# SimFlowCFD/RapidCFD-dev

Hardware: AMD Instinct MI355X
Metric: PCG iterations/s + HBM GB/s on 10M-cell lduMatrix at 1/2/4/8 MI355X (higher is better)
Workload: dtype f64

## Files before the change

### rapidcfd-dev_amd/csrc/engine.hip

```cpp
#include <hip/hip_ext.h>
#include "../../include/mi_ldu.h"
#include "kernels.hip.hpp"
#include "tiling.hpp"
#include "host_parallel.hpp"

#include <algorithm>
#include <atomic>
#include <cstdio>
#include <cstdlib>
#include <cstring>
#include <condition_variable>
#include <functional>
#include <map>
#include <set>
#include <mutex>
#include <string>
#include <thread>
#include <vector>

using namespace mi;
constexpr int HALO_NV = 6;

namespace {

thread_local std::string g_err;
int fail(int code, const std::string& msg) { g_err = msg; return code; }

#define HIPCHK(expr)                                                                          \
    do {                                                                                      \
        hipError_t e__ = (expr);                                                              \
        if (e__ != hipSuccess)                                                                \
            return fail(MI_ERR_DEVICE, std::string(#expr) + ": " + hipGetErrorString(e__));   \
    } while (0)
#define MICHK(expr) do { int r__ = (expr); if (r__ != MI_OK) return r__; } while (0)

template <class T>
struct DevBuf {
    T* p = nullptr;
    size_t n = 0;
    DevBuf() = default;
    DevBuf(const DevBuf&) = delete;
    DevBuf& operator=(const DevBuf&) = delete;
    ~DevBuf() { release(); }
    void release() { if (p) { (void)hipFree(p); p = nullptr; n = 0; } }
    int alloc(size_t count)
    {
        if (count == n && p) return MI_OK;
        release();
        if (hipMalloc((void**)&p, (count ? count : 1) * sizeof(T)) != hipSuccess) { p = nullptr; return fail(MI_ERR_ALLOC, "hipMalloc failed"); }
        n = count;
        return MI_OK;
    }
    template <class A>
    int upload(const std::vector<T, A>& v, hipStream_t s)
    {
        MICHK(alloc(v.size()));
        if (!v.empty()) HIPCHK(hipMemcpyAsync(p, v.data(), v.size() * sizeof(T), hipMemcpyHostToDevice, s));
        return MI_OK;
    }
};

int env_int(const char* name, int def)
{
    const char* v = getenv(name);
    return (v && *v) ? atoi(v) : def;
}

}

struct mi_ctx_s {
    int device = 0;
    hipStream_t stream = nullptr;
    bool ownStream = false;
    DevBuf<double> partial;
    DevBuf<double> scalars;
    DevBuf<PcgState> state;
    PcgState* hostState = nullptr;
    double* hostScal = nullptr;
    hipEvent_t ev0 = nullptr, ev1 = nullptr;
    hipStream_t sideStream = nullptr;
    hipEvent_t evSideGo = nullptr, evSideDone = nullptr;
    int amulBS = 0;
    int tileFlags = 0;
    int xcdRows = 1;
    int persist = 0;
    int nCU = 0;
    bool coarseLevelBuild = false;
    bool keepSlotTables = false;
    int attachEvents = 1;
    int fusePerm = 1;
    int deferPsi = 1;
    int fuseFinal = 0;
    int pcgFuseTest = 0;
    int pcgFuseRP = -1;
    int pcgPersist = 1;
    int64_t stats[12] = {};
    int persistGrid = 0;
    int persistShared = 0;
    int persistCoop = -1;
    uint64_t faultEpoch = 0;
    int winDirect = 1;
    int gamgGraphAttached = 1;
    int multiPipe = 1;
    int fusePrologue = 1;
    int pairAT = 1;
    struct mi_matrix_s* session = nullptr;
    int pcgBatch = 16, pcgGraph = -1, pbicgHostStepped = 0, gamgDeviceInvert = -1, gamgAlwaysAgglomerate = 0, gamgGraph = 1, gamgFuse = 1;
    std::set<const void*> ldsAttrSet;
    std::map<std::pair<const void*, size_t>, int> occCache;
};

struct mi_addr_s {
    mi_ctx_s* ctx = nullptr;
    TileLayout L;
    DevBuf<int32_t> e2c, c2e, tileCellStart, tileSlotStart, tileIfaceSlot0, tileHaloStart, haloCell, tileSliceStart, sliceEntryStart;
    DevBuf<uint32_t> entries, entries16;
    DevBuf<int32_t> sliceEntryStart16, tileSbStart;
    DevBuf<uint16_t> slotBase;
    bool compact = false;
    DevBuf<int32_t> slotFace, extSlot, interiorTiles, boundaryTiles, patchFaceCellsE, faceSlot, lowerAddr, upperAddr;
    DevBuf<int32_t> ownerStartC, losortStartC, losortC;
    DevBuf<uint32_t> row16; DevBuf<uint16_t> losort16; DevBuf<int32_t> rowEsc, rowEscStart;
    struct RowPlan { bool tiles = false; int bs = 256, blocks = 0, maxFaces = 0, capForced = 0; } rowPlan[2];
    DevBuf<double> relaxD0, relaxSumOff;
    DevBuf<uint8_t> setMask; DevBuf<double> setVal;
    Table<int32_t> lowerHost, upperHost;
    int32_t nInterior = 0, nBoundary = 0, nLocalPatches = 0;
    Table<char> patchIsLocal;
    DevBuf<int32_t> ifaceNbrCaller;
    DevBuf<int32_t> haloSrc;
    Table<Table<int32_t>> patchFaceCellsHost, patchNbrCellsHost;
    int64_t nEntries = 0, nHaloTot = 0;
    struct AmiPatch {
        int32_t patch = 0, nbrPatch = 0, n = 0, extOff = 0;
        Table<int32_t> transports, partCount;
        int32_t transport = -1, nPartner = 0;
        DevBuf<int32_t> start, cellE, ownE; DevBuf<double> w; bool hasLow = false;
        Table<int32_t> hStart, hAddr; Table<double> hW, hMagSf;
    };
    Table<AmiPatch*> ami;
    bool amiRemote = false;
    ~mi_addr_s() { for (AmiPatch* q : ami) delete q; }
    bool identity = false;
    const int32_t* perm() const { return identity ? nullptr : e2c.p; }
};

struct mi_dpcg_s { double *psi = nullptr, *src = nullptr, *pA = nullptr, *wA = nullptr, *rA = nullptr, *scal = nullptr, *send = nullptr; int precond = 0; };

struct mi_matrix_s {
    mi_addr_s* addr = nullptr;
    mi_dpcg_s dp;
    DevBuf<double> diagE, upE, lowE, rD, sumAE;
    bool asym = false, bound = false, rDValid = false, sumAValid = false;
    Table<double> patchFactor;
    uint64_t epoch = 0;
    Table<DevBuf<double>*> work;
    DevBuf<double> hist, tilePartial;
    DevBuf<PcgState> mstate; DevBuf<double> mpartial, mhist, mtilePartial; PcgState* mhostState = nullptr;
    DevBuf<double> persistScratch;
    uint64_t persistFaultEpoch = 0;
    DevBuf<double> persistZ;
    int histLen = 0;
    int pcgIt = 0, pcgPrecond = MI_PRECOND_DIAGONAL;
    bool pcgActive = false;
    bool pcgPReady = false;
    DevBuf<unsigned int> fusedBar;
    unsigned int fusedGen = 0;
    Table<hipEvent_t> evPool;
    hipGraphExec_t pcgGraph = nullptr;
    struct { int precond = -1, batch = 0, histLen = 0; const void* hist = nullptr; const void* psi = nullptr; } pcgGraphKey;
    bool gateDone = false;
    double *proY2 = nullptr, *proY3 = nullptr;
    const double *callerX = nullptr, *callerB = nullptr; double* callerY = nullptr;
    hipEvent_t kevStart = nullptr, kevStop = nullptr;
    struct mi_dpcg_comm_s* dpc = nullptr;
    DevBuf<double> sendBuf, dscal;
    ~mi_matrix_s();
    int vec(size_t k, double** out)
    {
        while (work.size() <= k) work.push_back(new DevBuf<double>());
        const size_t need = (size_t)addr->L.nCells + (size_t)addr->L.nExt;
        if (work[k]->n != need) {
            MICHK(work[k]->alloc(need));
            HIPCHK(hipMemsetAsync(work[k]->p, 0, need * sizeof(double), addr->ctx->stream));
        }
        *out = work[k]->p;
        return MI_OK;
    }
};

bool comm_remote(const mi_matrix_s* m);
bool comm_attached(const mi_matrix_s* m);
bool comm_any_ami(const mi_matrix_s* m);
bool comm_any_factor(const mi_matrix_s* m);
bool comm_any_compact(const mi_matrix_s* m);
bool matrix_has_factor(const mi_matrix_s* m);
void comm_inherit_factor_flag(mi_matrix_s* level, const mi_matrix_s* fine);
int64_t comm_n_global(const mi_matrix_s* m);
int comm_exchange_start(mi_matrix_s* m, const double* send, double* vec);
int comm_exchange_wait(mi_matrix_s* m);
int comm_allreduce(mi_matrix_s* m, double* dev, size_t n);
bool peer_halo_ready(const mi_matrix_s* m);
int peer_exchange_push(mi_matrix_s* m, const double* x);
int peer_exchange_pull(mi_matrix_s* m, double* x);
int peer_exchange_push_n(mi_matrix_s* m, int nv, const double* const* xs);
int peer_exchange_pull_n(mi_matrix_s* m, int nv, double* const* xs);
bool peer_win_direct(mi_matrix_s* m);
int peer_check(mi_matrix_s* m);
int dpcg_flush_if_fused(mi_matrix_s* m);
bool peer_reduce_ready(const mi_matrix_s* m);
int peer_globalize(mi_matrix_s* m, int n, double* const* P);
int pcg_solve_attached(mi_matrix_s* m, double* psi_io, const double* source, const mi_solver_controls* ctl, int precond,
                       mi_solver_perf* perf, double* hist_host, int32_t hist_len);

extern "C" const char* mi_last_error(void) { return g_err.c_str(); }

extern "C" int mi_device_available(void)
{
    int n = 0;
    if (hipGetDeviceCount(&n) != hipSuccess || n <= 0) return 0;
    hipDeviceProp_t prop;
    if (hipGetDeviceProperties(&prop, 0) != hipSuccess) return 0;
    return strncmp(prop.gcnArchName, "gfx950", 6) == 0 ? 1 : 0;
}

extern "C" int mi_ctx_create(int device, void* hip_stream, mi_ctx_t* out)
{
    if (!out) return fail(MI_ERR_ARG, "out is NULL");
    int n = 0;
    const hipError_t e0 = hipGetDeviceCount(&n);
    if (e0 != hipSuccess || n <= 0)
        return fail(MI_ERR_DEVICE, std::string("no HIP device visible: the engine has no CPU fallback (hipGetDeviceCount: ") + hipGetErrorString(e0) + ", " + std::to_string(n) + " devices)");
    if (device < 0 || device >= n) return fail(MI_ERR_ARG, "device index out of range");
    HIPCHK(hipSetDevice(device));
    hipDeviceProp_t prop;
    HIPCHK(hipGetDeviceProperties(&prop, device));
    if (strncmp(prop.gcnArchName, "gfx950", 6) != 0)
        return fail(MI_ERR_DEVICE, std::string("engine is built for gfx950 only, found ") + prop.gcnArchName);
    mi_ctx_s* c = new mi_ctx_s();
    c->device = device;
    if (hip_stream) c->stream = (hipStream_t)hip_stream;
    else { if (hipStreamCreate(&c->stream) != hipSuccess) { delete c; return fail(MI_ERR_DEVICE, "hipStreamCreate failed"); } c->ownStream = true; }
    int r = c->partial.alloc(4 * RG);
    if (r == MI_OK) r = c->scalars.alloc(16);
    if (r == MI_OK) r = c->state.alloc(1);
    if (r != MI_OK) { delete c; return r; }
    if (hipHostMalloc((void**)&c->hostState, sizeof(PcgState)) != hipSuccess ||
        hipHostMalloc((void**)&c->hostScal, 16 * sizeof(double)) != hipSuccess ||
        hipEventCreate(&c->ev0) != hipSuccess || hipEventCreate(&c->ev1) != hipSuccess) {
        delete c; return fail(MI_ERR_DEVICE, "pinned host / event allocation failed");
    }
    c->tileFlags = env_int("MI_TILE_FLAGS", 1);
    c->attachEvents = env_int("MI_EVENT_ATTACH", 1);
    c->persist = env_int("MI_TILE_PERSIST", 0);
    c->xcdRows = env_int("MI_XCD_ROWS", 1);
    c->deferPsi = env_int("MI_PCG_DEFER_PSI", 1);
    c->fusePerm = env_int("MI_FUSE_PERM", 1);
    { hipDeviceProp_t pr; if (hipGetDeviceProperties(&pr, device) == hipSuccess) c->nCU = pr.multiProcessorCount; }
    c->pairAT = env_int("MI_PBICG_PAIR", 1);
    c->fusePrologue = env_int("MI_FUSE_PROLOGUE", 1);
    c->multiPipe = env_int("MI_MULTI_PIPE", 1);
    c->winDirect = env_int("MI_WIN_DIRECT", 1); c->gamgGraphAttached = env_int("MI_GAMG_GRAPH_ATTACHED", 1);
    c->pcgPersist = env_int("MI_PCG_PERSIST", 1);
    c->pcgFuseRP = env_int("MI_PCG_FUSE_RP", 1) != 0 ? -1 : 0;
    c->persistGrid = env_int("MI_PERSIST_GRID", 0);
    c->persistShared = env_int("MI_PERSIST_SHARED", 0);
    c->fuseFinal = env_int("MI_PCG_FUSE_FINAL", 0);
    c->amulBS = env_int("MI_AMUL_BS", 0);
    c->pcgBatch = env_int("MI_PCG_BATCH", 16);
    if (c->pcgBatch < 1) c->pcgBatch = 1;
    c->pcgGraph = env_int("MI_PCG_GRAPH", -1); c->pbicgHostStepped = env_int("MI_PBICG_HOST_STEPPED", 0);
    c->gamgDeviceInvert = env_int("MI_GAMG_DEVICE_INVERT", -1); c->gamgAlwaysAgglomerate = env_int("MI_GAMG_ALWAYS_AGGLOMERATE", 0); c->gamgGraph = env_int("MI_GAMG_GRAPH", 1); c->gamgFuse = env_int("MI_GAMG_FUSE", 1);
    if (c->amulBS != 256 && c->amulBS != 512 && c->amulBS != 1024) c->amulBS = 0;
    *out = c;
    return MI_OK;
}

extern "C" int mi_ctx_destroy(mi_ctx_t c)
{
    if (!c) return MI_OK;
    (void)hipSetDevice(c->device);
    (void)hipStreamSynchronize(c->stream);
    if (c->hostState) (void)hipHostFree(c->hostState);
    if (c->hostScal) (void)hipHostFree(c->hostScal);
    if (c->ev0) (void)hipEventDestroy(c->ev0);
    if (c->ev1) (void)hipEventDestroy(c->ev1);
    if (c->sideStream) { (void)hipStreamSynchronize(c->sideStream); (void)hipStreamDestroy(c->sideStream); }
    if (c->evSideGo) (void)hipEventDestroy(c->evSideGo);
    if (c->evSideDone) (void)hipEventDestroy(c->evSideDone);
    if (c->ownStream) (void)hipStreamDestroy(c->stream);
    delete c;
    return MI_OK;
}

extern "C" int mi_ctx_synchronize(mi_ctx_t c)
{
    if (!c) return fail(MI_ERR_ARG, "ctx is NULL");
    HIPCHK(hipStreamSynchronize(c->stream));
    return MI_OK;
}

extern "C" int mi_ctx_set_option(mi_ctx_t c, const char* name, int32_t value)
{
    if (!c || !name) return fail(MI_ERR_ARG, "mi_ctx_set_option: bad argument");
    if (std::string(name) == "pcg_persist") { c->pcgPersist = value; return MI_OK; }
    if (std::string(name) == "pcg_fuse_rp") { c->pcgFuseRP = value != 0 ? -1 : 0; return MI_OK; }
    if (std::string(name) == "pcg_fuse_test") { c->pcgFuseTest = value; return MI_OK; }
    if (std::string(name) == "fuse_prologue") { c->fusePrologue = value; return MI_OK; }
    if (std::string(name) == "win_direct") { c->winDirect = value; return MI_OK; }
    if (std::string(name) == "gamg_graph_attached") { c->gamgGraphAttached = value; return MI_OK; }
    return fail(MI_ERR_ARG, "mi_ctx_set_option: unknown option");
}

extern "C" int mi_ctx_stat(mi_ctx_t c, int32_t which, int64_t* out)
{
    if (!c || !out || which < 0 || which >= (int32_t)(sizeof(c->stats) / sizeof(c->stats[0]))) return fail(MI_ERR_ARG, "mi_ctx_stat: bad argument");
    *out = c->stats[which];
    return MI_OK;
}

extern "C" int mi_addr_create_coupled(mi_ctx_t ctx, int32_t n_cells, int32_t n_faces,
                                      const int32_t* lower, const int32_t* upper, int32_t n_patches,
                                      const int32_t* patch_sizes, const int32_t* const* patch_face_cells,
                                      const int32_t* const* patch_nbr_cells, mi_addr_t* out);

extern "C" int mi_addr_create(mi_ctx_t ctx, int32_t n_cells, int32_t n_faces,
                              const int32_t* lower, const int32_t* upper, int32_t n_patches,
                              const int32_t* patch_sizes, const int32_t* const* patch_face_cells,
                              mi_addr_t* out)
{
    return mi_addr_create_coupled(ctx, n_cells, n_faces, lower, upper, n_patches, patch_sizes, patch_face_cells, nullptr, out);
}

static int addr_create_impl(mi_ctx_t ctx, int32_t n_cells, int32_t n_faces, const int32_t* lower, const int32_t* upper, int32_t n_patches,
                            const int32_t* patch_sizes, const int32_t* const* patch_face_cells, const int32_t* const* patch_nbr_cells,
                            bool ordered, int32_t n_tiles, const int32_t* tile_cell_start, mi_addr_t* out, TileLayout* prebuilt);

extern "C" int mi_addr_create_coupled(mi_ctx_t ctx, int32_t n_cells, int32_t n_faces,
                                      const int32_t* lower, const int32_t* upper, int32_t n_patches,
                                      const int32_t* patch_sizes, const int32_t* const* patch_face_cells,
                                      const int32_t* const* patch_nbr_cells, mi_addr_t* out)
{
    return addr_create_impl(ctx, n_cells, n_faces, lower, upper, n_patches, patch_sizes, patch_face_cells, patch_nbr_cells, false, 0, nullptr, out, nullptr);
}

extern "C" int mi_addr_create_ordered(mi_ctx_t ctx, int32_t n_cells, int32_t n_faces, const int32_t* lower, const int32_t* upper,
                                      int32_t n_patches, const int32_t* patch_sizes, const int32_t* const* patch_face_cells,
                                      const int32_t* const* patch_nbr_cells, int32_t n_tiles, const int32_t* tile_cell_start, mi_addr_t* out)
{
    if (tile_cell_start && n_tiles <= 0) return fail(MI_ERR_ARG, "mi_addr_create_ordered: n_tiles must be positive when tile_cell_start is given");
    return addr_create_impl(ctx, n_cells, n_faces, lower, upper, n_patches, patch_sizes, patch_face_cells, patch_nbr_cells, true, n_tiles, tile_cell_start, out, nullptr);
}

namespace {
struct AdoptedMesh {
    Table<int32_t> cellMap, faceMap, lower, upper, tileStart;
    Table<uint8_t> flipped;
    Table<Table<int32_t>> patchFaceCells, patchNbrCells;
};
std::string adopt_engine_order(int32_t n_cells, int32_t n_faces, const int32_t* lower, const int32_t* upper, int32_t n_patches, const int32_t* patch_sizes,
                               const int32_t* const* patch_face_cells, const int32_t* const* patch_nbr_cells, AdoptedMesh& M)
{
    TileLayout L;
    TileParams prm;
    prm.tileCells = env_int("MI_TILE_CELLS", 0) > 0 ? env_int("MI_TILE_CELLS", 0) : 1024;
    prm.slotCap = env_int("MI_TILE_SLOTS", 4094);
    prm.reorder = env_int("MI_TILE_REORDER", -1);
    prm.compact = false;
    const std::string err = build_tile_layout(n_cells, n_faces, lower, upper, n_patches, patch_sizes, patch_face_cells, prm, L, patch_nbr_cells);
    if (!err.empty()) return err;
    M.cellMap = L.e2c; M.tileStart = L.tileCellStart;
    const Table<int32_t>& o2n = L.c2e;
    Table<int32_t> lo((size_t)n_faces), up((size_t)n_faces);
    Table<uint8_t> fl((size_t)n_faces);
    for (int32_t f = 0; f < n_faces; ++f) {
        const int32_t a = o2n[(size_t)lower[f]], b = o2n[(size_t)upper[f]];
        fl[(size_t)f] = a > b; lo[(size_t)f] = a < b ? a : b; up[(size_t)f] = a < b ? b : a;
    }
    Table<int32_t> byUp((size_t)n_faces), cnt((size_t)n_cells + 1, 0);
    for (int32_t f = 0; f < n_faces; ++f) cnt[(size_t)up[(size_t)f] + 1]++;
    for (int32_t c = 0; c < n_cells; ++c) cnt[(size_t)c + 1] += cnt[(size_t)c];
    for (int32_t f = 0; f < n_faces; ++f) byUp[(size_t)cnt[(size_t)up[(size_t)f]]++] = f;
    std::fill(cnt.begin(), cnt.end(), 0);
    for (int32_t f = 0; f < n_faces; ++f) cnt[(size_t)lo[(size_t)f] + 1]++;
    for (int32_t c = 0; c < n_cells; ++c) cnt[(size_t)c + 1] += cnt[(size_t)c];
    M.faceMap.resize((size_t)n_faces);
    for (int32_t k = 0; k < n_faces; ++k) { const int32_t f = byUp[(size_t)k]; M.faceMap[(size_t)cnt[(size_t)lo[(size_t)f]]++] = f; }
    M.lower.resize((size_t)n_faces); M.upper.resize((size_t)n_faces); M.flipped.resize((size_t)n_faces);
    for (int32_t k = 0; k < n_faces; ++k) { const int32_t f = M.faceMap[(size_t)k]; M.lower[(size_t)k] = lo[(size_t)f]; M.upper[(size_t)k] = up[(size_t)f]; M.flipped[(size_t)k] = fl[(size_t)f]; }
    M.patchFaceCells.resize((size_t)n_patches); M.patchNbrCells.resize((size_t)n_patches);
    for (int32_t p = 0; p < n_patches; ++p) {
        for (int32_t i = 0; i < patch_sizes[p]; ++i) M.patchFaceCells[(size_t)p].push_back(o2n[(size_t)patch_face_cells[p][i]]);
        if (patch_nbr_cells && patch_nbr_cells[p]) for (int32_t i = 0; i < patch_sizes[p]; ++i) M.patchNbrCells[(size_t)p].push_back(o2n[(size_t)patch_nbr_cells[p][i]]);
    }
    return std::string();
}
void adopted_maps_out(const AdoptedMesh& M, int32_t* cell_map, int32_t* face_map, uint8_t* flipped, int32_t* lower_out, int32_t* upper_out)
{
    if (cell_map) memcpy(cell_map, M.cellMap.data(), sizeof(int32_t) * M.cellMap.size());
    if (face_map) memcpy(face_map, M.faceMap.data(), sizeof(int32_t) * M.faceMap.size());
    if (flipped) memcpy(flipped, M.flipped.data(), M.flipped.size());
    if (lower_out) memcpy(lower_out, M.lower.data(), sizeof(int32_t) * M.lower.size());
    if (upper_out) memcpy(upper_out, M.upper.data(), sizeof(int32_t) * M.upper.size());
}
}

extern "C" int mi_layout_adopt_host(int32_t n_cells, int32_t n_faces, const int32_t* lower, const int32_t* upper, int32_t n_patches, const int32_t* patch_sizes,
                                    const int32_t* const* patch_face_cells, const int32_t* const* patch_nbr_cells, int32_t* cell_new_to_old_out,
                                    int32_t* face_new_to_old_out, uint8_t* face_flipped_out, int32_t* lower_out, int32_t* upper_out, int32_t* n_tiles_out)
{
    if ((n_faces > 0 && (!lower || !upper)) || n_patches < 0) return fail(MI_ERR_ARG, "mi_layout_adopt_host: bad argument");
    AdoptedMesh M;
    const std::string err = adopt_engine_order(n_cells, n_faces, lower, upper, n_patches, patch_sizes, patch_face_cells, patch_nbr_cells, M);
    if (!err.empty()) return fail(MI_ERR_LIMIT, "mi_layout_adopt_host: " + err);
    adopted_maps_out(M, cell_new_to_old_out, face_new_to_old_out, face_flipped_out, lower_out, upper_out);
    if (n_tiles_out) *n_tiles_out = (int32_t)M.tileStart.size() - 1;
    return MI_OK;
}
extern "C" int mi_addr_create_adopted(mi_ctx_t ctx, int32_t n_cells, int32_t n_faces, const int32_t* lower, const int32_t* upper, int32_t n_patches,
                                      const int32_t* patch_sizes, const int32_t* const* patch_face_cells, const int32_t* const* patch_nbr_cells,
                                      int32_t* cell_new_to_old_out, int32_t* face_new_to_old_out, uint8_t* face_flipped_out, int32_t* lower_out, int32_t* upper_out,
                                      mi_addr_t* out)
{
    if (!ctx || !out || (n_faces > 0 && (!lower || !upper)) || n_patches < 0) return fail(MI_ERR_ARG, "mi_addr_create_adopted: bad argument");
    AdoptedMesh M;
    const std::string err = adopt_engine_order(n_cells, n_faces, lower, upper, n_patches, patch_sizes, patch_face_cells, patch_nbr_cells, M);
    if (!err.empty()) return fail(MI_ERR_LIMIT, "mi_addr_create_adopted: " + err);
    Table<const int32_t*> pfc((size_t)n_patches), pnb((size_t)n_patches, nullptr);
    bool anyNbr = false;
    for (int32_t p = 0; p < n_patches; ++p) {
        pfc[(size_t)p] = M.patchFaceCells[(size_t)p].data();
        if (patch_nbr_cells && patch_nbr_cells[p]) { pnb[(size_t)p] = M.patchNbrCells[(size_t)p].data(); anyNbr = true; }
    }
    MICHK(addr_create_impl(ctx, n_cells, n_faces, M.lower.data(), M.upper.data(), n_patches, patch_sizes, pfc.data(), anyNbr ? pnb.data() : nullptr, true,
                           (int32_t)M.tileStart.size() - 1, M.tileStart.data(), out, nullptr));
    adopted_maps_out(M, cell_new_to_old_out, face_new_to_old_out, face_flipped_out, lower_out, upper_out);
    return MI_OK;
}

extern "C" int mi_addr_tile_starts(mi_addr_t a, int32_t* tile_cell_start_out)
{
    if (!a || !tile_cell_start_out) return fail(MI_ERR_ARG, "mi_addr_tile_starts: bad argument");
    memcpy(tile_cell_start_out, a->L.tileCellStart.data(), sizeof(int32_t) * a->L.tileCellStart.size());
    return MI_OK;
}
extern "C" int mi_addr_is_ordered(mi_addr_t a) { return a && a->identity ? 1 : 0; }

static TileParams addr_tile_params(mi_ctx_t ctx, int32_t n_cells, bool coarse, bool ordered, int32_t n_tiles, const int32_t* tile_cell_start);
static int addr_create_impl(mi_ctx_t ctx, int32_t n_cells, int32_t n_faces, const int32_t* lower, const int32_t* upper, int32_t n_patches,
                            const int32_t* patch_sizes, const int32_t* const* patch_face_cells, const int32_t* const* patch_nbr_cells,
                            bool ordered, int32_t n_tiles, const int32_t* tile_cell_start, mi_addr_t* out, TileLayout* prebuilt);
static TileParams addr_tile_params(mi_ctx_t ctx, int32_t n_cells, bool coarse, bool ordered, int32_t n_tiles, const int32_t* tile_cell_start)
{
    TileParams prm;
    prm.tileCells = env_int("MI_TILE_CELLS", 0);
    if (prm.tileCells <= 0) {
        const int target = (coarse && env_int("MI_SMALL_TILES", 1)) ? (int)(((int64_t)n_cells / std::max(1, ctx->nCU) + 63) / 64 * 64) : 1024;
        prm.tileCells = std::min(1024, std::max(128, target));
    }
    prm.slotCap = env_int("MI_TILE_SLOTS", 4094);
    prm.reorder = env_int("MI_TILE_REORDER", -1);
    prm.compact = env_int("MI_ENTRY16", 0) != 0;
    prm.keepOrder = ordered; prm.givenTileStart = tile_cell_start; prm.nGivenTiles = n_tiles;
    return prm;
}
static int addr_create_impl(mi_ctx_t ctx, int32_t n_cells, int32_t n_faces, const int32_t* lower, const int32_t* upper, int32_t n_patches,
                            const int32_t* patch_sizes, const int32_t* const* patch_face_cells, const int32_t* const* patch_nbr_cells,
                            bool ordered, int32_t n_tiles, const int32_t* tile_cell_start, mi_addr_t* out, TileLayout* prebuilt)
{
    if (!ctx || !out || (n_faces > 0 && (!lower || !upper)) || n_patches < 0)
        return fail(MI_ERR_ARG, "mi_addr_create: bad argument");
    HIPCHK(hipSetDevice(ctx->device));
    mi_addr_s* a = new mi_addr_s();
    a->ctx = ctx;
    TileParams prm;
    prm.tileCells = env_int("MI_TILE_CELLS", 0);
    if (prm.tileCells <= 0) {
        const int target = (ctx->coarseLevelBuild && env_int("MI_SMALL_TILES", 1)) ? (int)(((int64_t)n_cells / std::max(1, ctx->nCU) + 63) / 64 * 64) : 1024;
        prm.tileCells = std::min(1024, std::max(128, target));
    }
    prm.slotCap = env_int("MI_TILE_SLOTS", 4094);
    prm.reorder = env_int("MI_TILE_REORDER", -1);
    prm.compact = env_int("MI_ENTRY16", 0) != 0;
    prm.keepOrder = ordered; prm.givenTileStart = tile_cell_start; prm.nGivenTiles = n_tiles;
#ifdef MI_TIMING
    auto ta__ = std::chrono::steady_clock::now();
    auto ta_tick = [&](const char* what) { auto n = std::chrono::steady_clock::now(); if (n_cells > 1000000) fprintf(stderr, "[addr] %-28s %.4f s\n", what, std::chrono::duration<double>(n - ta__).count()); ta__ = n; };
#endif
    if (prebuilt) a->L = std::move(*prebuilt);
    else {
    const std::string err = build_tile_layout(n_cells, n_faces, lower, upper, n_patches, patch_sizes, patch_face_cells, prm, a->L, patch_nbr_cells);
    if (!err.empty()) { delete a; return fail(MI_ERR_LIMIT, "mi_addr_create: " + err); }
    }
#ifdef MI_TIMING
    ta_tick("tile layout (host)");
#endif
    a->identity = true;
    for (int32_t e = 0; e < n_cells; ++e) if (a->L.e2c[(size_t)e] != e) { a->identity = false; break; }
    a->nLocalPatches = 0;
    a->patchIsLocal.assign((size_t)std::max(n_patches, 0), 0);
    if (patch_nbr_cells) for (int32_t p = 0; p < n_patches; ++p) if (patch_nbr_cells[p]) { a->nLocalPatches++; a->patchIsLocal[(size_t)p] = 1; }
    TileLayout& L = a->L;
    hipStream_t s = ctx->stream;
    int r = MI_OK;
#define UP(buf, vec) if (r == MI_OK) r = a->buf.upload(vec, s)
    UP(e2c, L.e2c); UP(c2e, L.c2e); UP(tileCellStart, L.tileCellStart); UP(tileSlotStart, L.tileSlotStart); UP(tileIfaceSlot0, L.tileIfaceSlot0);
    UP(tileHaloStart, L.tileHaloStart); UP(haloCell, L.haloCell); UP(tileSliceStart, L.tileSliceStart);
    a->compact = L.compact;
    if (L.compact) { UP(sliceEntryStart16, L.sliceEntryStart16); UP(entries16, L.entries16); UP(slotBase, L.slotBase); UP(tileSbStart, L.tileSbStart); }
    else { UP(sliceEntryStart, L.sliceEntryStart); UP(entries, L.entries); }
    UP(slotFace, L.slotFace);
    UP(extSlot, L.extSlot); UP(interiorTiles, L.interiorTiles); UP(boundaryTiles, L.boundaryTiles);
    UP(patchFaceCellsE, L.patchFaceCellsE); UP(faceSlot, L.faceSlot);
#undef UP
    if (r != MI_OK) { delete a; return r; }
    if (hipStreamSynchronize(s) != hipSuccess) { delete a; return fail(MI_ERR_DEVICE, "upload failed"); }
#ifdef MI_TIMING
    ta_tick("uploads + synchronise");
#endif
    a->nInterior = (int32_t)L.interiorTiles.size();
    a->nBoundary = (int32_t)L.boundaryTiles.size();
    a->nEntries = (int64_t)(L.compact ? L.entries16.size() : L.entries.size());
    a->nHaloTot = (int64_t)L.haloCell.size();
    a->lowerHost.resize((size_t)n_faces); a->upperHost.resize((size_t)n_faces);
    mi::parallel_blocks(n_faces, 1 << 20, [&](int64_t b, int64_t e, int) {
        std::memcpy(a->lowerHost.data() + b, lower + b, sizeof(int32_t) * (size_t)(e - b));
        std::memcpy(a->upperHost.data() + b, upper + b, sizeof(int32_t) * (size_t)(e - b));
    });
    a->patchFaceCellsHost.resize((size_t)n_patches); a->patchNbrCellsHost.resize((size_t)n_patches);
    for (int32_t p = 0; p < n_patches; ++p) {
        a->patchFaceCellsHost[(size_t)p].assign(patch_face_cells[p], patch_face_cells[p] + patch_sizes[p]);
        if (a->patchIsLocal[(size_t)p]) a->patchNbrCellsHost[(size_t)p].assign(patch_nbr_cells[p], patch_nbr_cells[p] + patch_sizes[p]);
    }
    {
        Table<int32_t> slotFace, faceSlot;
        if (!ctx->keepSlotTables) { slotFace.swap(L.slotFace); faceSlot.swap(L.faceSlot); }
        mi::free_in_background(L.entries, L.entries16, L.sliceEntryStart16, L.slotBase, slotFace, L.haloCell, L.sliceEntryStart, faceSlot);
        L.entries = Table<uint32_t>(); L.entries16 = Table<uint32_t>(); L.sliceEntryStart16 = Table<int32_t>(); L.slotBase = Table<uint16_t>();
        L.haloCell = Table<int32_t>(); L.sliceEntryStart = Table<int32_t>();
    }
#ifdef MI_TIMING
    ta_tick("host copies + frees");
#endif
    *out = a;
    return MI_OK;
}

extern "C" int mi_addr_destroy(mi_addr_t a) { delete a; return MI_OK; }

extern "C" int mi_addr_set_ami_patch(mi_addr_t a, int32_t patch, int32_t nbr_patch, const int32_t* start, const int32_t* address, const double* weights,
                                     const uint8_t* low_weight)
{
    if (!a || patch < 0 || patch >= a->L.nPatches || nbr_patch < 0 || nbr_patch >= a->L.nPatches)
        return fail(MI_ERR_ARG, "mi_addr_set_ami_patch: bad argument");
    if (a->patchIsLocal[(size_t)patch]) return fail(MI_ERR_ARG, "mi_addr_set_ami_patch: the patch must be created without neighbour cells (ext region), once");
    if ((start || address || weights) && !(start && address && weights)) return fail(MI_ERR_ARG, "mi_addr_set_ami_patch: start, address and weights go together");
    HIPCHK(hipSetDevice(a->ctx->device));
    const Table<int32_t>& mine = a->patchFaceCellsHost[(size_t)patch];
    const Table<int32_t>& theirs = a->patchFaceCellsHost[(size_t)nbr_patch];
    const int32_t n = (int32_t)mine.size(), nn = (int32_t)theirs.size();
    Table<int32_t> st((size_t)n + 1, 0), ce, own;
    Table<double> w;
    if (!start) {
        if (n != nn) return fail(MI_ERR_ARG, "mi_addr_set_ami_patch: one-to-one coupling needs patches of equal size");
        ce.resize((size_t)n); w.assign((size_t)n, 1.0);
        for (int32_t i = 0; i < n; ++i) { st[(size_t)i + 1] = i + 1; ce[i] = a->L.c2e[(size_t)theirs[i]]; }
    } else {
        if (start[0] != 0) return fail(MI_ERR_ARG, "mi_addr_set_ami_patch: start[0] must be 0");
        for (int32_t i = 0; i < n; ++i) if (start[i + 1] < start[i]) return fail(MI_ERR_ARG, "mi_addr_set_ami_patch: start must be non-decreasing");
        const int32_t na = start[n];
        ce.resize((size_t)na); w.assign(weights, weights + na);
        for (int32_t k = 0; k < na; ++k) {
            if (address[k] < 0 || address[k] >= nn) return fail(MI_ERR_ARG, "mi_addr_set_ami_patch: address outside the neighbour patch");
            ce[k] = a->L.c2e[(size_t)theirs[(size_t)address[k]]];
        }
        st.assign(start, start + n + 1);
    }
    mi_addr_s::AmiPatch* q = new mi_addr_s::AmiPatch();
    q->patch = patch; q->nbrPatch = nbr_patch; q->n = n; q->extOff = a->L.patchOffset[(size_t)patch];
    q->hStart = st; q->hW = w;
    if (start) q->hAddr.assign(address, address + start[n]); else { q->hAddr.resize((size_t)n); for (int32_t i = 0; i < n; ++i) q->hAddr[i] = i; }
    if (low_weight) {
        own.assign((size_t)n, -1);
        for (int32_t i = 0; i < n; ++i) if (low_weight[i]) { own[i] = a->L.c2e[(size_t)mine[i]]; q->hasLow = true; }
    }
    hipStream_t s = a->ctx->stream;
    int r = q->start.upload(st, s);
    if (r == MI_OK && !ce.empty()) r = q->cellE.upload(ce, s);
    if (r == MI_OK && !w.empty()) r = q->w.upload(w, s);
    if (r == MI_OK && q->hasLow) r = q->ownE.upload(own, s);
    if (r != MI_OK) { delete q; return r; }
    HIPCHK(hipStreamSynchronize(s));
    a->ami.push_back(q);
    a->patchIsLocal[(size_t)patch] = 2;
    a->nLocalPatches++;
    return MI_OK;
}

int ami_remote_impl(mi_addr_s* a, int32_t patch, const Table<int32_t>& transports, const Table<int32_t>& partCount, const int32_t* start,
                    const int32_t* addrSlot, const int32_t* addrFace, const int32_t* hAddrConcat, const double* weights, const uint8_t* low_weight)
{
    const char* me = "mi_addr_set_ami_patch_remote";
    if (!a || patch < 0 || patch >= a->L.nPatches || transports.empty() || transports.size() != partCount.size() || !start || !weights) return fail(MI_ERR_ARG, std::string(me) + ": bad argument");
    if (a->patchIsLocal[(size_t)patch]) return fail(MI_ERR_ARG, std::string(me) + ": the cyclicAMI patch must be created without neighbour cells (an ext region)");
    int32_t total = 0;
    for (size_t q = 0; q < transports.size(); ++q) {
        const int32_t t = transports[q];
        if (t < 0 || t >= a->L.nPatches || t == patch || a->patchIsLocal[(size_t)t]) return fail(MI_ERR_ARG, std::string(me) + ": a transport patch must be a processor patch of this addressing (created without neighbour cells)");
        for (size_t r = 0; r < q; ++r) if (transports[r] == t) return fail(MI_ERR_ARG, std::string(me) + ": a transport patch is listed twice");
        const int32_t nT = a->L.patchOffset[(size_t)t + 1] - a->L.patchOffset[(size_t)t];
// ... 1720 lines not shown
```

### rapidcfd-dev_amd/csrc/pcg_fused.inc

```
namespace mi {

constexpr int FUSED_HR = 5;
constexpr int FUSED_PF = 3;
constexpr int FUSED_LP = 2544;
constexpr int FUSED_BAR_WORDS = BAR_LINE * (RG + 64) + RG + 64;
constexpr int FUSED_PEND_AT = BAR_LINE * (RG + 64);
constexpr long long FUSED_WAIT_POLLS = 1000;

struct FusedArgs {
    PcgState* st;
    int it;
    const double* partial2;
    double *partial3, *partial1;
    const double *wA, *rD;
    double *pA, *psi, *rA;
    int64_t n;
    double* hist; int histLen;
    unsigned int* bar; unsigned int gen;
    long long maxPolls;
    int testMode;
};

__device__ __forceinline__ void st_agent(double* p, double v)
{
    __hip_atomic_store(reinterpret_cast<unsigned long long*>(p), (unsigned long long)__double_as_longlong(v), __ATOMIC_RELAXED, __HIP_MEMORY_SCOPE_AGENT);
}
__device__ __forceinline__ double ld_agent(const double* p)
{
    return __longlong_as_double((long long)__hip_atomic_load(reinterpret_cast<const unsigned long long*>(p), __ATOMIC_RELAXED, __HIP_MEMORY_SCOPE_AGENT));
}
__device__ __forceinline__ double sum_partials_agent(const double* partial, double* red)
{
    double v = 0;
#pragma unroll
    for (int k = 0; k < RG / RB; ++k) v += ld_agent(partial + threadIdx.x + k * RB);
    return block_sum<RB>(v, red);
}

__device__ __forceinline__ void fused_arrive(unsigned int* bar, unsigned int target, int* flag)
{
    __builtin_amdgcn_fence(__ATOMIC_RELEASE, "workgroup");
    __builtin_amdgcn_s_waitcnt(0);
    if (threadIdx.x == 0) *flag = 1;
    __syncthreads();
    if (blockIdx.x != 0 && threadIdx.x == 0) __hip_atomic_store(&bar[blockIdx.x * BAR_LINE], target, __ATOMIC_RELAXED, __HIP_MEMORY_SCOPE_AGENT);
}
__device__ __forceinline__ bool fused_wait(unsigned int* bar, unsigned int target, long long maxPolls, int testMode, int* flag)
{
    const unsigned int b = blockIdx.x, tid = threadIdx.x;
    if (b == 0) {
        if (testMode & 2) { if (tid == 0) *flag = 0; }
        else
        for (unsigned int w = tid; w < (unsigned int)RG; w += RB) {
            if (w == 0) continue;
            long long polls = 0;
            while (__hip_atomic_load(&bar[w * BAR_LINE], __ATOMIC_RELAXED, __HIP_MEMORY_SCOPE_AGENT) != target) {
                if (++polls > maxPolls) { *flag = 0; break; }
                __builtin_amdgcn_s_sleep(1);
            }
        }
        __syncthreads();
        if (*flag != 0 && tid < 64) __hip_atomic_store(&bar[(RG + tid) * BAR_LINE], target, __ATOMIC_RELAXED, __HIP_MEMORY_SCOPE_AGENT);
    } else {
        if (tid == 0) {
            const unsigned int* line = &bar[(RG + (b & 63u)) * BAR_LINE];
            long long polls = 0;
            if ((testMode & 1) && b % 3u == 1u) *flag = 0;
            else
            while (__hip_atomic_load(line, __ATOMIC_RELAXED, __HIP_MEMORY_SCOPE_AGENT) != target) {
                if (++polls > 2 * maxPolls) { *flag = 0; break; }
                __builtin_amdgcn_s_sleep(1);
            }
        }
        __syncthreads();
    }
    __builtin_amdgcn_fence(__ATOMIC_ACQUIRE, "workgroup");
    const bool ok = *flag != 0;
    __syncthreads();
    return ok;
}

struct FusedScalars { double res, wArA, beta; bool conv, cont; };
template <bool AGENT>
__device__ __forceinline__ FusedScalars fused_scalars(const PcgState* st, int it, const double* partial3, const double* partial1, double wArAold, double* red)
{
    FusedScalars q;
    q.res = (AGENT ? sum_partials_agent(partial3, red) : sum_partials(partial3, red)) / st->normFactor;
    q.conv = sp_converged(st, q.res);
    q.cont = (it < st->maxIter && !q.conv) || (it + 1 < st->minIter);
    q.wArA = AGENT ? sum_partials_agent(partial1, red) : sum_partials(partial1, red);
    q.beta = q.wArA / wArAold;
    return q;
}
__device__ __forceinline__ void fused_close(PcgState* st, int it, double alpha, double wApA, const FusedScalars& q, double* hist, int histLen)
{
    st->alpha = alpha; st->wApA = wApA;
    st->finalResidual = q.res;
    if (it + 1 < histLen) hist[it + 1] = q.res;
    st->nIterations = it + 1;
    st->it = it + 1;
    st->converged = q.conv;
    if (q.cont) st->wArA[(it + 1) & 1] = q.wArA; else st->done = 1;
    st->pApplyItP1 = st->rItP1;
}

template <int PMODE>
__global__ __launch_bounds__(RB, 8) void k_pcg_fused_r_p(FusedArgs a)
{
    extern __shared__ double2 zLds[];
    __shared__ double red[RB / 64];
    __shared__ int flag;
    PcgState* __restrict__ st = a.st;
    if (st->done) return;
    const int it = a.it;
    const unsigned int b = blockIdx.x, tid = threadIdx.x;
    const bool lead = b == 0 && tid == 0;
    const double wApA = sum_partials(a.partial2, red);
    if (fabs(wApA) / st->normFactor < SP_VSMALL) {
        if (tid == 0) a.partial3[b] = -1.0;
        if (lead) { st->singular = 1; st->done = 1; }
        return;
    }
    const double wArAold = st->wArA[it & 1];
    const double alpha = wArAold / wApA;
    const Chunk ck = my_chunk(a.n);
    const double* __restrict__ wA = a.wA + ck.lo; const double* __restrict__ rD = a.rD + (PMODE == 1 ? ck.lo : 0);
    double* __restrict__ rA = a.rA + ck.lo; double* __restrict__ pA = a.pA + ck.lo; double* __restrict__ psi = a.psi + ck.lo;
    const int len = (int)(ck.hi - ck.lo), np = len >> 1;
    const bool oddTail = (len & 1) && tid == 0;
    double acc0 = 0, acc1 = 0, d0 = 0, d1 = 0;
    double2 zr[FUSED_HR];
    double zTail = 0.0;
    auto residual2 = [&](int i) -> double2 {
        const double2 w = ld2_stream(wA, i);
        double2 r = ld2(rA, i);
        r.x = fma(-alpha, w.x, r.x); r.y = fma(-alpha, w.y, r.y);
        st2(rA, i, r); acc0 += fabs(r.x); acc1 += fabs(r.y);
        double2 z = r;
        if (PMODE == 1) { const double2 d = ld2_rd(rD, i); z.x = d.x * r.x; z.y = d.y * r.y; }
        d0 = fma(z.x, r.x, d0); d1 = fma(z.y, r.y, d1);
        return z;
    };
#pragma unroll
    for (int k = 0; k < FUSED_HR; ++k) {
        const int q = (int)tid + k * RB;
        zr[k] = make_double2(0.0, 0.0);
        if (q < np) zr[k] = residual2(2 * q);
    }
    for (int q = (int)tid + FUSED_HR * RB; q < np; q += RB) {
        const double2 z = residual2(2 * q);
        const int l = q - FUSED_HR * RB;
        if (l < FUSED_LP) zLds[l] = z;
    }
    if (oddTail) {
        const int i = len - 1;
        const double r = fma(-alpha, wA[i], rA[i]); rA[i] = r; acc0 += fabs(r);
        zTail = (PMODE == 1) ? rD[i] * r : r;
        d0 = fma(zTail, r, d0);
    }
    const double t = block_sum<RB>(acc0 + acc1, red);
    const double u = block_sum<RB>(d0 + d1, red);
    if (tid == 0) { st_agent(a.partial3 + b, t); st_agent(a.partial1 + b, u); }
    fused_arrive(a.bar, a.gen, &flag);
    double2 pf[FUSED_PF];
#pragma unroll
    for (int k = 0; k < FUSED_PF; ++k) {
        const int q = (int)tid + k * RB;
        pf[k] = make_double2(0.0, 0.0);
        if (q < np) {
            const int i = 2 * q;
            pf[k] = ld2(pA, i);
            double2 x = ld2_stream(psi, i);
            x.x = fma(alpha, pf[k].x, x.x); x.y = fma(alpha, pf[k].y, x.y);
            st2_stream(psi, i, x);
        }
    }
    if (!fused_wait(a.bar, a.gen, a.maxPolls, a.testMode, &flag)) {
        if (tid == 0) __hip_atomic_store(&a.bar[FUSED_PEND_AT + b], 1u, __ATOMIC_RELAXED, __HIP_MEMORY_SCOPE_AGENT);
        if (lead) __hip_atomic_store(&a.bar[FUSED_PEND_AT + RG], 1u, __ATOMIC_RELAXED, __HIP_MEMORY_SCOPE_AGENT);
        return;
    }
    const FusedScalars sc = fused_scalars<true>(st, it, a.partial3, a.partial1, wArAold, red);
    const bool cont = sc.cont;
    const double beta = sc.beta;
    auto direction2 = [&](int i, double2 z) {
        const double2 p = ld2(pA, i);
        double2 x = ld2_stream(psi, i);
        x.x = fma(alpha, p.x, x.x); x.y = fma(alpha, p.y, x.y);
        st2_stream(psi, i, x);
        if (cont) st2(pA, i, make_double2(fma(beta, p.x, z.x), fma(beta, p.y, z.y)));
    };
#pragma unroll
    for (int k = 0; k < FUSED_HR; ++k) {
        const int q = (int)tid + k * RB;
        if (q < np) {
            if (k < FUSED_PF) { if (cont) st2(pA, 2 * q, make_double2(fma(beta, pf[k].x, zr[k].x), fma(beta, pf[k].y, zr[k].y))); }
            else direction2(2 * q, zr[k]);
        }
    }
    for (int q = (int)tid + FUSED_HR * RB; q < np; q += RB) {
        const int l = q - FUSED_HR * RB, i = 2 * q;
        double2 z;
        if (l < FUSED_LP) z = zLds[l];
        else { z = ld2(rA, i); if (PMODE == 1) { const double2 d = ld2_rd(rD, i); z.x = d.x * z.x; z.y = d.y * z.y; } }
        direction2(i, z);
    }
    if (oddTail) {
        const int i = len - 1;
        const double p = pA[i];
        psi[i] = fma(alpha, p, psi[i]);
        if (cont) pA[i] = fma(beta, p, zTail);
    }
    if (lead) fused_close(st, it, alpha, wApA, sc, a.hist, a.histLen);
}

template <int PMODE>
__global__ __launch_bounds__(RB) void k_pcg_fused_finish(FusedArgs a)
{
    __shared__ double red[RB / 64];
    const unsigned int b = blockIdx.x, tid = threadIdx.x;
    unsigned int* pend = a.bar + FUSED_PEND_AT;
    PcgState* __restrict__ st = a.st;
    if (b == 0 && tid == 0 && st->rItP1 >= a.it) st->pApplyItP1 = a.it;
    const bool mine = pend[b] != 0u, closing = b == 0 && pend[RG] != 0u;
    if (!mine && !closing) return;
    const int it = a.it;
    const double wApA = sum_partials(a.partial2, red);
    const double wArAold = st->wArA[it & 1];
    const double alpha = wArAold / wApA;
    const FusedScalars sc = fused_scalars<false>(st, it, a.partial3, a.partial1, wArAold, red);
    if (mine) {
        const Chunk ck = my_chunk(a.n);
        const double* __restrict__ rD = a.rD + (PMODE == 1 ? ck.lo : 0); const double* __restrict__ rA = a.rA + ck.lo;
        double* __restrict__ pA = a.pA + ck.lo; double* __restrict__ psi = a.psi + ck.lo;
        const int len = (int)(ck.hi - ck.lo), np = len >> 1;
        for (int q = (int)tid; q < np; q += RB) {
            const int i = 2 * q;
            double2 z = ld2(rA, i);
            if (PMODE == 1) { const double2 d = ld2_rd(rD, i); z.x = d.x * z.x; z.y = d.y * z.y; }
            const double2 p = ld2(pA, i);
            if (q >= FUSED_PF * RB) {
                double2 x = ld2(psi, i);
                x.x = fma(alpha, p.x, x.x); x.y = fma(alpha, p.y, x.y);
                st2(psi, i, x);
            }
            if (sc.cont) st2(pA, i, make_double2(fma(sc.beta, p.x, z.x), fma(sc.beta, p.y, z.y)));
        }
        if ((len & 1) && tid == 0) {
            const int i = len - 1;
            const double z = (PMODE == 1) ? rD[i] * rA[i] : rA[i];
            const double p = pA[i];
            psi[i] = fma(alpha, p, psi[i]);
            if (sc.cont) pA[i] = fma(sc.beta, p, z);
        }
    }
    __syncthreads();
    if (tid == 0) { pend[b] = 0u; if (closing) { fused_close(st, it, alpha, wApA, sc, a.hist, a.histLen); pend[RG] = 0u; } }
}

}

namespace {

bool pcg_fused_rp_usable(const mi_matrix_s* m, int precond)
{
    const mi_ctx_s* c = m->addr->ctx;
    return c->pcgFuseRP != 0 && !comm_attached(m) && (precond == MI_PRECOND_DIAGONAL || precond == MI_PRECOND_NONE) && !c->fuseFinal;
}

int pcg_fused_rp_launch(mi_matrix_s* m, int it, int precond)
{
    mi_addr_s* a = m->addr;
    mi_ctx_s* c = a->ctx;
    hipStream_t s = c->stream;
    const void* fn = precond == MI_PRECOND_DIAGONAL ? (const void*)k_pcg_fused_r_p<1> : (const void*)k_pcg_fused_r_p<2>;
    const size_t lds = sizeof(double2) * (size_t)FUSED_LP;
    if (c->pcgFuseRP < 0) {
        int perCU = 0, nCU = 0;
        (void)hipDeviceGetAttribute(&nCU, hipDeviceAttributeMultiprocessorCount, c->device);
        for (const void* f : {(const void*)k_pcg_fused_r_p<1>, (const void*)k_pcg_fused_r_p<2>}) {
            int q = 0;
            if (hipOccupancyMaxActiveBlocksPerMultiprocessor(&q, f, RB, lds) != hipSuccess) { (void)hipGetLastError(); q = 0; }
            perCU = (f == (const void*)k_pcg_fused_r_p<1>) ? q : std::min(perCU, q);
        }
        c->pcgFuseRP = ((int64_t)perCU * nCU >= RG) ? 1 : 0;
        if (!c->pcgFuseRP) return MI_ERR_UNSUPPORTED;
    }
    if (m->fusedBar.n < (size_t)FUSED_BAR_WORDS) {
        MICHK(m->fusedBar.alloc((size_t)FUSED_BAR_WORDS));
        HIPCHK(hipMemsetAsync(m->fusedBar.p, 0, sizeof(unsigned int) * (size_t)FUSED_BAR_WORDS, s));
        m->fusedGen = 0;
    }
    if (++m->fusedGen == 0u) {
        HIPCHK(hipMemsetAsync(m->fusedBar.p, 0, sizeof(unsigned int) * BAR_LINE * (size_t)(RG + 64), s));
        m->fusedGen = 1u;
    }
    FusedArgs A;
    A.st = c->state.p; A.it = it;
    A.partial1 = c->partial.p; A.partial2 = c->partial.p + RG; A.partial3 = c->partial.p + 2 * RG;
    double *psi, *pA, *wA, *rA;
    MICHK(m->vec(3, &psi)); MICHK(m->vec(5, &pA)); MICHK(m->vec(6, &wA)); MICHK(m->vec(7, &rA));
    A.wA = wA; A.rD = m->rD.p; A.pA = pA; A.psi = psi; A.rA = rA; A.n = a->L.nCells;
    A.hist = m->hist.p; A.histLen = m->histLen;
    A.bar = m->fusedBar.p; A.gen = m->fusedGen;
    static const long long polls = (long long)env_int("MI_PCG_FUSE_POLLS", (int)FUSED_WAIT_POLLS);
    A.maxPolls = polls;
    A.testMode = c->pcgFuseTest;
    void* args[1] = {&A};
    static const int coop = env_int("MI_PCG_FUSE_COOP", 0);
    if (coop) {
        if (hipLaunchCooperativeKernel(fn, dim3(RG), dim3(RB), args, (unsigned int)lds, s) != hipSuccess) {
            (void)hipGetLastError();
            c->pcgFuseRP = 0;
            return MI_ERR_UNSUPPORTED;
        }
    } else if (precond == MI_PRECOND_DIAGONAL) k_pcg_fused_r_p<1><<<RG, RB, lds, s>>>(A);
    else k_pcg_fused_r_p<2><<<RG, RB, lds, s>>>(A);
    if (precond == MI_PRECOND_DIAGONAL) k_pcg_fused_finish<1><<<RG, RB, 0, s>>>(A); else k_pcg_fused_finish<2><<<RG, RB, 0, s>>>(A);
    HIPCHK(hipGetLastError());
    c->stats[4] += 1;
    return MI_OK;
}

}
```

Baseline: 3670.

## Retire pending fused PCG chunks in last-arriving block instead of separate finish kernel

Adds a two-level arrival ticket (per-XCD counters plus a global one) so the last block of the fused residual/preconditioner kernel finishes any chunks whose blocks timed out in the grid wait, and closes the iteration. The separate finish kernel launch is dropped when retire mode is on (the default), removing one launch and its full-grid pass per PCG iteration. The cost is extra atomics on every block's exit, and serial processing of pending chunks by a single block when timeouts occur. It also moves pApplyItP1 bookkeeping to the kernel start.

```diff
diff --git a/rapidcfd-dev_amd/csrc/engine.hip b/rapidcfd-dev_amd/csrc/engine.hip
--- a/rapidcfd-dev_amd/csrc/engine.hip
+++ b/rapidcfd-dev_amd/csrc/engine.hip
@@ -94,6 +94,7 @@
     int pcgFuseTest = 0;
     int pcgFuseRP = -1;
     int pcgPersist = 1;
+    int pcgFusedRetire = 1;
     int64_t stats[12] = {};
     int persistGrid = 0;
     int persistShared = 0;
@@ -263,6 +264,7 @@
     c->winDirect = env_int("MI_WIN_DIRECT", 1); c->gamgGraphAttached = env_int("MI_GAMG_GRAPH_ATTACHED", 1);
     c->pcgPersist = env_int("MI_PCG_PERSIST", 1);
     c->pcgFuseRP = env_int("MI_PCG_FUSE_RP", 1) != 0 ? -1 : 0;
+    c->pcgFusedRetire = env_int("MI_PCG_FUSE_RETIRE", 1);
     c->persistGrid = env_int("MI_PERSIST_GRID", 0);
     c->persistShared = env_int("MI_PERSIST_SHARED", 0);
     c->fuseFinal = env_int("MI_PCG_FUSE_FINAL", 0);
@@ -306,6 +308,7 @@
     if (std::string(name) == "pcg_persist") { c->pcgPersist = value; return MI_OK; }
     if (std::string(name) == "pcg_fuse_rp") { c->pcgFuseRP = value != 0 ? -1 : 0; return MI_OK; }
     if (std::string(name) == "pcg_fuse_test") { c->pcgFuseTest = value; return MI_OK; }
+    if (std::string(name) == "pcg_fuse_retire") { c->pcgFusedRetire = value; return MI_OK; }
     if (std::string(name) == "fuse_prologue") { c->fusePrologue = value; return MI_OK; }
     if (std::string(name) == "win_direct") { c->winDirect = value; return MI_OK; }
     if (std::string(name) == "gamg_graph_attached") { c->gamgGraphAttached = value; return MI_OK; }
diff --git a/rapidcfd-dev_amd/csrc/pcg_fused.inc b/rapidcfd-dev_amd/csrc/pcg_fused.inc
--- a/rapidcfd-dev_amd/csrc/pcg_fused.inc
+++ b/rapidcfd-dev_amd/csrc/pcg_fused.inc
@@ -3,8 +3,11 @@
 constexpr int FUSED_HR = 5;
 constexpr int FUSED_PF = 3;
 constexpr int FUSED_LP = 2544;
-constexpr int FUSED_BAR_WORDS = BAR_LINE * (RG + 64) + RG + 64;
 constexpr int FUSED_PEND_AT = BAR_LINE * (RG + 64);
+constexpr int FUSED_RET_AT = FUSED_PEND_AT + RG + 64;
+constexpr int FUSED_ANY_AT = FUSED_RET_AT + 9 * BAR_LINE;
+constexpr int FUSED_BAR_WORDS = FUSED_ANY_AT + BAR_LINE;
+static_assert(FUSED_RET_AT % BAR_LINE == 0, "the ticket's counters sit on their own 64-byte lines");
 constexpr long long FUSED_WAIT_POLLS = 1000;
 
 struct FusedArgs {
@@ -19,6 +22,7 @@
     unsigned int* bar; unsigned int gen;
     long long maxPolls;
     int testMode;
+    int retire;
 };
 
 __device__ __forceinline__ void st_agent(double* p, double v)
@@ -104,17 +108,109 @@
     st->pApplyItP1 = st->rItP1;
 }
 
+__device__ __forceinline__ bool last_arrival(unsigned int* ctr, unsigned int* flag)
+{
+    __syncthreads();
+    if (threadIdx.x == 0) {
+        __builtin_amdgcn_fence(__ATOMIC_RELEASE, "workgroup");
+        __builtin_amdgcn_s_waitcnt(0);
+        const unsigned int G = gridDim.x, x = blockIdx.x & 7u;
+        const unsigned int nx = (G - x + 7u) >> 3, nS = G < 8u ? G : 8u;
+        unsigned int last = 0u;
+        if (__hip_atomic_fetch_add(&ctr[x * BAR_LINE], 1u, __ATOMIC_RELAXED, __HIP_MEMORY_SCOPE_AGENT) == nx - 1u) {
+            __hip_atomic_store(&ctr[x * BAR_LINE], 0u, __ATOMIC_RELAXED, __HIP_MEMORY_SCOPE_AGENT);
+            if (__hip_atomic_fetch_add(&ctr[8u * BAR_LINE], 1u, __ATOMIC_RELAXED, __HIP_MEMORY_SCOPE_AGENT) == nS - 1u) {
+                __hip_atomic_store(&ctr[8u * BAR_LINE], 0u, __ATOMIC_RELAXED, __HIP_MEMORY_SCOPE_AGENT);
+                last = 1u;
+            }
+        }
+        *flag = last;
+    }
+    __syncthreads();
+    __builtin_amdgcn_fence(__ATOMIC_ACQUIRE, "workgroup");
+    return *flag != 0u;
+}
+
+template <class T>
+__device__ __forceinline__ T* opaque(T* p)
+{
+    asm volatile("" : "+s"(p));
+    return p;
+}
+
+template <int PMODE>
+__device__ __forceinline__ void fused_finish_chunk(const FusedArgs& a, int64_t lo, int64_t hi, double alpha, const FusedScalars& sc)
+{
+    const unsigned int tid = threadIdx.x;
+    const double* __restrict__ rD = a.rD + (PMODE == 1 ? lo : 0); const double* __restrict__ rA = a.rA + lo;
+    double* __restrict__ pA = a.pA + lo; double* __restrict__ psi = a.psi + lo;
+    const int len = (int)(hi - lo), np = len >> 1;
+    for (int q = (int)tid; q < np; q += RB) {
+        const int i = 2 * q;
+        double2 z = ld2(rA, i);
+        if (PMODE == 1) { const double2 d = ld2_rd(rD, i); z.x = d.x * z.x; z.y = d.y * z.y; }
+        const double2 p = ld2(pA, i);
+        if (q >= FUSED_PF * RB) {
+            double2 x = ld2(psi, i);
+            x.x = fma(alpha, p.x, x.x); x.y = fma(alpha, p.y, x.y);
+            st2(psi, i, x);
+        }
+        if (sc.cont) st2(pA, i, make_double2(fma(sc.beta, p.x, z.x), fma(sc.beta, p.y, z.y)));
+    }
+    if ((len & 1) && tid == 0) {
+        const int i = len - 1;
+        const double z = (PMODE == 1) ? rD[i] * rA[i] : rA[i];
+        const double p = pA[i];
+        psi[i] = fma(alpha, p, psi[i]);
+        if (sc.cont) pA[i] = fma(sc.beta, p, z);
+    }
+}
+
+template <int PMODE>
+__device__ __forceinline__ void fused_retire(const FusedArgs& a, unsigned int* zw, double* red, unsigned int* lastFlag)
+{
+    if (!last_arrival(a.bar + FUSED_RET_AT, lastFlag)) return;
+    unsigned int* anyPend = a.bar + FUSED_ANY_AT;
+    if (__hip_atomic_load(anyPend, __ATOMIC_RELAXED, __HIP_MEMORY_SCOPE_AGENT) == 0u) return;
+    __builtin_amdgcn_fence(__ATOMIC_ACQUIRE, "agent");
+    const unsigned int tid = threadIdx.x;
+    unsigned int* pend = a.bar + FUSED_PEND_AT;
+    for (unsigned int c = tid; c <= (unsigned int)RG; c += RB) zw[c] = __hip_atomic_load(&pend[c], __ATOMIC_RELAXED, __HIP_MEMORY_SCOPE_AGENT);
+    __syncthreads();
+    PcgState* __restrict__ st = a.st;
+    const int it = a.it;
+    const double wApA = sum_partials(opaque(a.partial2), red);
+    const double wArAold = st->wArA[it & 1];
+    const double alpha = wArAold / wApA;
+    const FusedScalars sc = fused_scalars<true>(st, it, opaque(a.partial3), opaque(a.partial1), wArAold, red);
+    int64_t chunk = (a.n + RG - 1) / RG;
+    chunk = (chunk + 1) & ~int64_t(1);
+    for (unsigned int c = 0; c < (unsigned int)RG; ++c) {
+        if (zw[c] == 0u) continue;
+        int64_t lo = (int64_t)c * chunk; if (lo > a.n) lo = a.n;
+        int64_t hi = lo + chunk; if (hi > a.n) hi = a.n;
+        fused_finish_chunk<PMODE>(a, lo, hi, alpha, sc);
+        if (tid == 0) pend[c] = 0u;
+    }
+    if (tid == 0) {
+        if (zw[RG] != 0u) { fused_close(st, it, alpha, wApA, sc, a.hist, a.histLen); pend[RG] = 0u; }
+        *anyPend = 0u;
+    }
+}
+
 template <int PMODE>
 __global__ __launch_bounds__(RB, 8) void k_pcg_fused_r_p(FusedArgs a)
 {
     extern __shared__ double2 zLds[];
     __shared__ double red[RB / 64];
     __shared__ int flag;
+    __shared__ unsigned int lastFlag;
     PcgState* __restrict__ st = a.st;
-    if (st->done) return;
     const int it = a.it;
     const unsigned int b = blockIdx.x, tid = threadIdx.x;
     const bool lead = b == 0 && tid == 0;
+    if (a.retire && lead && st->rItP1 >= it) st->pApplyItP1 = it;
+    if (st->done) return;
     const double wApA = sum_partials(a.partial2, red);
     if (fabs(wApA) / st->normFactor < SP_VSMALL) {
         if (tid == 0) a.partial3[b] = -1.0;
@@ -130,7 +226,6 @@
     const bool oddTail = (len & 1) && tid == 0;
     double acc0 = 0, acc1 = 0, d0 = 0, d1 = 0;
     double2 zr[FUSED_HR];
-    double zTail = 0.0;
     auto residual2 = [&](int i) -> double2 {
         const double2 w = ld2_stream(wA, i);
         double2 r = ld2(rA, i);
@@ -155,7 +250,7 @@
     if (oddTail) {
         const int i = len - 1;
         const double r = fma(-alpha, wA[i], rA[i]); rA[i] = r; acc0 += fabs(r);
-        zTail = (PMODE == 1) ? rD[i] * r : r;
+        const double zTail = (PMODE == 1) ? rD[i] * r : r;
         d0 = fma(zTail, r, d0);
     }
     const double t = block_sum<RB>(acc0 + acc1, red);
@@ -175,43 +270,50 @@
             st2_stream(psi, i, x);
         }
     }
-    if (!fused_wait(a.bar, a.gen, a.maxPolls, a.testMode, &flag)) {
+    const bool stay = fused_wait(a.bar, a.gen, a.maxPolls, a.testMode, &flag);
+    if (!stay) {
         if (tid == 0) __hip_atomic_store(&a.bar[FUSED_PEND_AT + b], 1u, __ATOMIC_RELAXED, __HIP_MEMORY_SCOPE_AGENT);
         if (lead) __hip_atomic_store(&a.bar[FUSED_PEND_AT + RG], 1u, __ATOMIC_RELAXED, __HIP_MEMORY_SCOPE_AGENT);
-        return;
-    }
-    const FusedScalars sc = fused_scalars<true>(st, it, a.partial3, a.partial1, wArAold, red);
-    const bool cont = sc.cont;
-    const double beta = sc.beta;
-    auto direction2 = [&](int i, double2 z) {
-        const double2 p = ld2(pA, i);
-        double2 x = ld2_stream(psi, i);
-        x.x = fma(alpha, p.x, x.x); x.y = fma(alpha, p.y, x.y);
-        st2_stream(psi, i, x);
-        if (cont) st2(pA, i, make_double2(fma(beta, p.x, z.x), fma(beta, p.y, z.y)));
-    };
+        if (a.retire) {
+            if (tid == 0) __hip_atomic_store(&a.bar[FUSED_ANY_AT], 1u, __ATOMIC_RELAXED, __HIP_MEMORY_SCOPE_AGENT);
+            __syncthreads();
+            if (tid == 0) __builtin_amdgcn_fence(__ATOMIC_RELEASE, "agent");
+        }
+    } else {
+        const FusedScalars sc = fused_scalars<true>(st, it, a.partial3, a.partial1, wArAold, red);
+        const bool cont = sc.cont;
+        const double beta = sc.beta;
+        auto direction2 = [&](int i, double2 z) {
+            const double2 p = ld2(pA, i);
+            double2 x = ld2_stream(psi, i);
+            x.x = fma(alpha, p.x, x.x); x.y = fma(alpha, p.y, x.y);
+            st2_stream(psi, i, x);
+            if (cont) st2(pA, i, make_double2(fma(beta, p.x, z.x), fma(beta, p.y, z.y)));
+        };
 #pragma unroll
-    for (int k = 0; k < FUSED_HR; ++k) {
-        const int q = (int)tid + k * RB;
-        if (q < np) {
-            if (k < FUSED_PF) { if (cont) st2(pA, 2 * q, make_double2(fma(beta, pf[k].x, zr[k].x), fma(beta, pf[k].y, zr[k].y))); }
-            else direction2(2 * q, zr[k]);
-        }
-    }
-    for (int q = (int)tid + FUSED_HR * RB; q < np; q += RB) {
-        const int l = q - FUSED_HR * RB, i = 2 * q;
-        double2 z;
-        if (l < FUSED_LP) z = zLds[l];
-        else { z = ld2(rA, i); if (PMODE == 1) { const double2 d = ld2_rd(rD, i); z.x = d.x * z.x; z.y = d.y * z.y; } }
-        direction2(i, z);
-    }
-    if (oddTail) {
-        const int i = len - 1;
-        const double p = pA[i];
-        psi[i] = fma(alpha, p, psi[i]);
-        if (cont) pA[i] = fma(beta, p, zTail);
-    }
-    if (lead) fused_close(st, it, alpha, wApA, sc, a.hist, a.histLen);
+        for (int k = 0; k < FUSED_HR; ++k) {
+            const int q = (int)tid + k * RB;
+            if (q < np) {
+                if (k < FUSED_PF) { if (cont) st2(pA, 2 * q, make_double2(fma(beta, pf[k].x, zr[k].x), fma(beta, pf[k].y, zr[k].y))); }
+                else direction2(2 * q, zr[k]);
+            }
+        }
+        for (int q = (int)tid + FUSED_HR * RB; q < np; q += RB) {
+            const int l = q - FUSED_HR * RB, i = 2 * q;
+            double2 z;
+            if (l < FUSED_LP) z = zLds[l];
+            else { z = ld2(rA, i); if (PMODE == 1) { const double2 d = ld2_rd(rD, i); z.x = d.x * z.x; z.y = d.y * z.y; } }
+            direction2(i, z);
+        }
+        if (oddTail) {
+            const int i = len - 1;
+            const double p = pA[i];
+            psi[i] = fma(alpha, p, psi[i]);
+            if (cont) pA[i] = fma(beta, p, (PMODE == 1) ? rD[i] * rA[i] : rA[i]);
+        }
+        if (lead) fused_close(st, it, alpha, wApA, sc, a.hist, a.histLen);
+    }
+    if (a.retire) fused_retire<PMODE>(a, reinterpret_cast<unsigned int*>(zLds), red, &lastFlag);
 }
 
 template <int PMODE>
@@ -231,28 +333,7 @@
     const FusedScalars sc = fused_scalars<false>(st, it, a.partial3, a.partial1, wArAold, red);
     if (mine) {
         const Chunk ck = my_chunk(a.n);
-        const double* __restrict__ rD = a.rD + (PMODE == 1 ? ck.lo : 0); const double* __restrict__ rA = a.rA + ck.lo;
-        double* __restrict__ pA = a.pA + ck.lo; double* __restrict__ psi = a.psi + ck.lo;
-        const int len = (int)(ck.hi - ck.lo), np = len >> 1;
-        for (int q = (int)tid; q < np; q += RB) {
-            const int i = 2 * q;
-            double2 z = ld2(rA, i);
-            if (PMODE == 1) { const double2 d = ld2_rd(rD, i); z.x = d.x * z.x; z.y = d.y * z.y; }
-            const double2 p = ld2(pA, i);
-            if (q >= FUSED_PF * RB) {
-                double2 x = ld2(psi, i);
-                x.x = fma(alpha, p.x, x.x); x.y = fma(alpha, p.y, x.y);
-                st2(psi, i, x);
-            }
-            if (sc.cont) st2(pA, i, make_double2(fma(sc.beta, p.x, z.x), fma(sc.beta, p.y, z.y)));
-        }
-        if ((len & 1) && tid == 0) {
-            const int i = len - 1;
-            const double z = (PMODE == 1) ? rD[i] * rA[i] : rA[i];
-            const double p = pA[i];
-            psi[i] = fma(alpha, p, psi[i]);
-            if (sc.cont) pA[i] = fma(sc.beta, p, z);
-        }
+        fused_finish_chunk<PMODE>(a, ck.lo, ck.hi, alpha, sc);
     }
     __syncthreads();
     if (tid == 0) { pend[b] = 0u; if (closing) { fused_close(st, it, alpha, wApA, sc, a.hist, a.histLen); pend[RG] = 0u; } }
@@ -306,6 +387,7 @@
     static const long long polls = (long long)env_int("MI_PCG_FUSE_POLLS", (int)FUSED_WAIT_POLLS);
     A.maxPolls = polls;
     A.testMode = c->pcgFuseTest;
+    A.retire = c->pcgFusedRetire != 0 ? 1 : 0;
     void* args[1] = {&A};
     static const int coop = env_int("MI_PCG_FUSE_COOP", 0);
     if (coop) {
@@ -316,7 +398,7 @@
         }
     } else if (precond == MI_PRECOND_DIAGONAL) k_pcg_fused_r_p<1><<<RG, RB, lds, s>>>(A);
     else k_pcg_fused_r_p<2><<<RG, RB, lds, s>>>(A);
-    if (precond == MI_PRECOND_DIAGONAL) k_pcg_fused_finish<1><<<RG, RB, 0, s>>>(A); else k_pcg_fused_finish<2><<<RG, RB, 0, s>>>(A);
+    if (!A.retire) { if (precond == MI_PRECOND_DIAGONAL) k_pcg_fused_finish<1><<<RG, RB, 0, s>>>(A); else k_pcg_fused_finish<2><<<RG, RB, 0, s>>>(A); }
     HIPCHK(hipGetLastError());
     c->stats[4] += 1;
     return MI_OK;
```

Measured after the change: 3681 (median of 6 runs). About the same (+0.3%).
